# bit-bots/SoccerDiffusion

Hardware: AMD Instinct MI355X
Metric: denoised joint-trajectories/s (50-step DDIM, H=100, J=20) (higher is better)
Workload: dtype f32 (operands split into fp16 hi+lo, 3 fp16 MFMAs per product at every site, fp32 accumulate: 22-bit operands; single noise prediction vs the fp64 oracle 8e-7 on these weights and 2e-6 on weights stressed to |logit| ~ 60 (tests/test_gpu_denoiser.py::test_mode3_noise_prediction_single_step); valid fo; 1 GPU; BASELINE.json configs[2]: 50-step DDIM sampling, B=4096 parallel rollouts per GPU, transformer denoiser d=256 L=4 heads=4, horizon T=100, J=20, memory M=11 (10 context tokens + step token); one step = one full rollout; the timed region issues the rollout's launches eagerly.  Kernel selection: sampler mode 3 (--sampler-mode); batch_per_gpu=4096, ddim_steps=50, horizon=100, joints=20, hidden_dim=256, decoder_layers=4, parallelism=dp1 (independent rollouts, no collective)

## Files before the change

soccerdiffusion_amd/csrc/sd_common.h:

```cpp
#ifndef SD_COMMON_H
#define SD_COMMON_H

#include <hip/hip_runtime.h>
#include <stdint.h>
#include <stdio.h>
#include <atomic>
#include <type_traits>
#include <vector>

#include "../../include/soccerdiffusion_hip.h"

typedef float f32x16 __attribute__((ext_vector_type(16)));
typedef float f32x4 __attribute__((ext_vector_type(4)));

#define SD_LN_EPS 1e-5f

#ifndef SD_PLAIN_STORES
#define SD_PLAIN_STORES 0
#endif
#if SD_PLAIN_STORES
#define SD_NT_STORE(v, p) (*(p) = (v))
#else
#define SD_NT_STORE(v, p) __builtin_nontemporal_store((v), (p))
#endif
// ... 2 lines not shown

#define SD_CHECK_LAUNCH(name)                                 \
    do {                                                      \
        hipError_t e_ = hipGetLastError();                    \
        if (e_ != hipSuccess) return fail((int)e_, name);     \
    } while (0)
#define SD_LAUNCH(...)                    \
    do {                                  \
        (void)hipGetLastError();          \
        hipLaunchKernelGGL(__VA_ARGS__);  \
    } while (0)

struct DevFlag {
    static constexpr int MAX_DEV = 64;
    std::atomic<bool> f[MAX_DEV];
    DevFlag() { for (auto &x : f) x.store(false, std::memory_order_relaxed); }
    static int dev() {
        int d = 0;
        if (hipGetDevice(&d) != hipSuccess || d < 0 || d >= MAX_DEV) d = 0;
        return d;
    }
    bool operator!() const { return !f[dev()].load(std::memory_order_acquire); }
    DevFlag &operator=(bool v) {
        f[dev()].store(v, std::memory_order_release);
        return *this;
    }
};

struct ProfRec { int cls; hipEvent_t a, b; };
struct ProfScope {
    bool on;
    ProfRec rec;
    hipStream_t st;
    ProfScope(int cls, hipStream_t s);
    ~ProfScope();
};

__device__ __forceinline__ float wave_sum(float v) {
#pragma unroll
    for (int o = 32; o > 0; o >>= 1) v += __shfl_xor(v, o, 64);
    return v;
}
__device__ __forceinline__ float wave_max(float v) {
#pragma unroll
    for (int o = 32; o > 0; o >>= 1) v = fmaxf(v, __shfl_xor(v, o, 64));
    return v;
}

__device__ __forceinline__ float row16_sum(float v) {
    v += __builtin_bit_cast(float, __builtin_amdgcn_update_dpp(0, __builtin_bit_cast(int, v), 0x128, 0xF, 0xF, false));
    v += __builtin_bit_cast(float, __builtin_amdgcn_update_dpp(0, __builtin_bit_cast(int, v), 0x124, 0xF, 0xF, false));
    v += __builtin_bit_cast(float, __builtin_amdgcn_update_dpp(0, __builtin_bit_cast(int, v), 0x122, 0xF, 0xF, false));
    v += __builtin_bit_cast(float, __builtin_amdgcn_update_dpp(0, __builtin_bit_cast(int, v), 0x121, 0xF, 0xF, false));
    return v;
}
__device__ __forceinline__ float row16_max(float v) {
    v = fmaxf(v, __builtin_bit_cast(float, __builtin_amdgcn_update_dpp(0, __builtin_bit_cast(int, v), 0x128, 0xF, 0xF, false)));
    v = fmaxf(v, __builtin_bit_cast(float, __builtin_amdgcn_update_dpp(0, __builtin_bit_cast(int, v), 0x124, 0xF, 0xF, false)));
    v = fmaxf(v, __builtin_bit_cast(float, __builtin_amdgcn_update_dpp(0, __builtin_bit_cast(int, v), 0x122, 0xF, 0xF, false)));
    v = fmaxf(v, __builtin_bit_cast(float, __builtin_amdgcn_update_dpp(0, __builtin_bit_cast(int, v), 0x121, 0xF, 0xF, false)));
    return v;
}

__device__ __forceinline__ void quad_transpose(float &x0, float &x1, float &x2, float &x3, int lane) {
    const bool o1 = lane & 1, o2 = lane & 2;
    float ta = o1 ? x0 : x1, tb = o1 ? x2 : x3;
    ta = __builtin_bit_cast(float, __builtin_amdgcn_update_dpp(0, __builtin_bit_cast(int, ta), 0xB1, 0xF, 0xF, false));
    tb = __builtin_bit_cast(float, __builtin_amdgcn_update_dpp(0, __builtin_bit_cast(int, tb), 0xB1, 0xF, 0xF, false));
    if (o1) { x0 = ta; x2 = tb; } else { x1 = ta; x3 = tb; }
    float tc = o2 ? x0 : x2, td = o2 ? x1 : x3;
    tc = __builtin_bit_cast(float, __builtin_amdgcn_update_dpp(0, __builtin_bit_cast(int, tc), 0x4E, 0xF, 0xF, false));
    td = __builtin_bit_cast(float, __builtin_amdgcn_update_dpp(0, __builtin_bit_cast(int, td), 0x4E, 0xF, 0xF, false));
    if (o2) { x0 = tc; x1 = td; } else { x2 = tc; x3 = td; }
}

__device__ __forceinline__ float gelu_erf(float u) { return 0.5f * u * (1.0f + erff(u * 0.70710678118654752440f)); }

__device__ __forceinline__ float gelu_erf_fast(float u) {
    const float z = u * 0.70710678118654752440f, a = fabsf(z);
    const float t = __builtin_amdgcn_rcpf(fmaf(0.5f, a, 1.0f));
    float p = 0.17087277f;
    p = fmaf(p, t, -0.82215223f);
    p = fmaf(p, t, 1.48851587f);
    p = fmaf(p, t, -1.13520398f);
    p = fmaf(p, t, 0.27886807f);
    p = fmaf(p, t, -0.18628806f);
    p = fmaf(p, t, 0.09678418f);
    p = fmaf(p, t, 0.37409196f);
    p = fmaf(p, t, 1.00002368f);
    p = fmaf(p, t, -1.26551223f);
    const float e = t * __builtin_amdgcn_exp2f(fmaf(-a, a, p) * 1.44269504088896340736f);
    return 0.5f * u * (z >= 0.f ? 2.0f - e : e);
}

__device__ __forceinline__ float gelu_grad_fast(float u) {
    const float z = u * 0.70710678118654752440f, a = fabsf(z);
    const float t = __builtin_amdgcn_rcpf(fmaf(0.5f, a, 1.0f));
    float p = 0.17087277f;
    p = fmaf(p, t, -0.82215223f);
    p = fmaf(p, t, 1.48851587f);
    p = fmaf(p, t, -1.13520398f);
    p = fmaf(p, t, 0.27886807f);
    p = fmaf(p, t, -0.18628806f);
    p = fmaf(p, t, 0.09678418f);
    p = fmaf(p, t, 0.37409196f);
    p = fmaf(p, t, 1.00002368f);
    p = fmaf(p, t, -1.26551223f);
    const float g = __builtin_amdgcn_exp2f(-a * a * 1.44269504088896340736f);
    const float e = 0.5f * t * g * __builtin_amdgcn_exp2f(p * 1.44269504088896340736f);
    return (z >= 0.f ? 1.0f - e : e) + u * 0.39894228040143267794f * g;
}

typedef _Float16 f16;
typedef _Float16 f16x4 __attribute__((ext_vector_type(4)));
typedef _Float16 f16x8 __attribute__((ext_vector_type(8)));

typedef float f32x2 __attribute__((ext_vector_type(2)));
__device__ __forceinline__ f32x2 gelu_erf_fast2(f32x2 u) {
    const f32x2 z = u * 0.70710678118654752440f;
    const f32x2 a = {fabsf(z[0]), fabsf(z[1])};
    const f32x2 d = a * 0.5f + 1.0f;
    const f32x2 t = {__builtin_amdgcn_rcpf(d[0]), __builtin_amdgcn_rcpf(d[1])};
    f32x2 p = {0.17087277f, 0.17087277f};
    p = p * t + (-0.82215223f);
    p = p * t + 1.48851587f;
    p = p * t + (-1.13520398f);
    p = p * t + 0.27886807f;
    p = p * t + (-0.18628806f);
    p = p * t + 0.09678418f;
    p = p * t + 0.37409196f;
    p = p * t + 1.00002368f;
    p = p * t + (-1.26551223f);
    const f32x2 x = (p - a * a) * 1.44269504088896340736f;
    const f32x2 e = {t[0] * __builtin_amdgcn_exp2f(x[0]), t[1] * __builtin_amdgcn_exp2f(x[1])};
    const f32x2 w = {z[0] >= 0.f ? 2.0f - e[0] : e[0], z[1] >= 0.f ? 2.0f - e[1] : e[1]};
    return u * 0.5f * w;
}

__device__ __forceinline__ f32x2 gelu_erf_as2(f32x2 u) {
    const f32x2 z = f32x2{fabsf(u[0]), fabsf(u[1])} * 0.70710678118654752440f;
    const f32x2 d = z * 0.3275911f + 1.0f;
    const f32x2 t = {__builtin_amdgcn_rcpf(d[0]), __builtin_amdgcn_rcpf(d[1])};
    f32x2 p = t * 1.061405429f + (-1.453152027f);
    p = p * t + 1.421413741f;
    p = p * t + (-0.284496736f);
    p = p * t + 0.254829592f;
    p = p * t;
    const f32x2 x = z * z * (-1.44269504088896340736f);
    const f32x2 e = {p[0] * __builtin_amdgcn_exp2f(x[0]), p[1] * __builtin_amdgcn_exp2f(x[1])};
    const f32x2 hu = u * 0.5f;
    return f32x2{u[0] >= 0.f ? fmaf(-hu[0], e[0], u[0]) : hu[0] * e[0], u[1] >= 0.f ? fmaf(-hu[1], e[1], u[1]) : hu[1] * e[1]};
}

__device__ __forceinline__ void f16_split4(const f32x4 &x, float scale, f16x4 &h, f16x4 &l) {
#pragma unroll
    for (int e = 0; e < 4; ++e) {
        const float v = x[e] * scale;
        h[e] = (f16)v;
        l[e] = (f16)(v - (float)h[e]);
    }
}

typedef __fp16 fp16x2_t __attribute__((ext_vector_type(2)));
__device__ __forceinline__ void f16_split4_pk(const f32x4 &x, float scale, f16x4 &h, f16x4 &l) {
    const f32x2 a = f32x2{x[0], x[1]} * scale, b = f32x2{x[2], x[3]} * scale;
    const fp16x2_t ha = __builtin_amdgcn_cvt_pkrtz(a[0], a[1]), hb = __builtin_amdgcn_cvt_pkrtz(b[0], b[1]);
    const f32x2 ra = a - f32x2{(float)ha[0], (float)ha[1]}, rb = b - f32x2{(float)hb[0], (float)hb[1]};
    const fp16x2_t la = __builtin_amdgcn_cvt_pkrtz(ra[0], ra[1]), lb = __builtin_amdgcn_cvt_pkrtz(rb[0], rb[1]);
    typedef unsigned u32x2 __attribute__((ext_vector_type(2)));
    h = __builtin_bit_cast(f16x4, u32x2{__builtin_bit_cast(unsigned, ha), __builtin_bit_cast(unsigned, hb)});
    l = __builtin_bit_cast(f16x4, u32x2{__builtin_bit_cast(unsigned, la), __builtin_bit_cast(unsigned, lb)});
}

__device__ __forceinline__ float f16_scale_from_bits(unsigned maxbits) {
    const unsigned eb = (maxbits >> 23) & 0xffu;
    const unsigned sbits = (267u - eb) << 23;
    return (eb >= 14u && eb != 255u) ? __builtin_bit_cast(float, sbits) : 1.0f;
}

struct DropoutArgs {
    unsigned thresh;
    float scale;
    unsigned seed_lo, seed_hi, site_lo, site_hi;
    const unsigned *epoch;
};
extern const unsigned *g_dropout_epoch;

static inline DropoutArgs make_dropout(float p, uint64_t seed, uint64_t site) {
    DropoutArgs a;
    double t = (double)p * 4294967296.0;
    a.thresh = p <= 0.f ? 0u : (t >= 4294967295.0 ? 4294967295u : (unsigned)t);
    a.scale = p <= 0.f ? 1.0f : 1.0f / (1.0f - p);
    a.seed_lo = (unsigned)seed; a.seed_hi = (unsigned)(seed >> 32);
    a.site_lo = (unsigned)site; a.site_hi = (unsigned)(site >> 32);
    a.epoch = g_dropout_epoch;
    return a;
}

__device__ __forceinline__ void philox4x32_7(unsigned c0, unsigned c1, unsigned c2, unsigned c3, unsigned k0, unsigned k1,
                                              unsigned (&w)[4]) {
#pragma unroll
    for (int i = 0; i < 7; ++i) {
        const unsigned long p0 = (unsigned long)0xD2511F53u * (unsigned long)c0, p1 = (unsigned long)0xCD9E8D57u * (unsigned long)c2;
        const unsigned hi0 = (unsigned)(p0 >> 32), lo0 = (unsigned)p0, hi1 = (unsigned)(p1 >> 32), lo1 = (unsigned)p1;
        c0 = hi1 ^ c1 ^ k0;
        c1 = lo1;
        c2 = hi0 ^ c3 ^ k1;
        c3 = lo0;
        k0 += 0x9E3779B9u;
        k1 += 0xBB67AE85u;
    }
    w[0] = c0; w[1] = c1; w[2] = c2; w[3] = c3;
}

__device__ __forceinline__ f32x4 dropout_quad(const DropoutArgs &a, unsigned long quad) {
#ifdef SD_ABL_NOPHILOX
    return f32x4{a.scale, a.scale, a.scale, a.scale} + (float)(quad == 0x123456789ul);
#endif
    unsigned w[4];
    philox4x32_7((unsigned)quad, (unsigned)(quad >> 32), a.site_lo, a.site_hi, a.seed_lo, a.seed_hi + (a.epoch ? *a.epoch : 0u), w);
    f32x4 m;
#pragma unroll
    for (int e = 0; e < 4; ++e) m[e] = w[e] >= a.thresh ? a.scale : 0.f;
    return m;
}

struct PinArgs {
    const float *x0, *noise;
    const int *rows;
};

struct HoldArgs {
    const float *x0, *noise;
    const int *mask;
};

struct MultistepArgs {
    float *hist;
    float w;
};

struct LimitArgs {
    const float *lo, *hi;
    int reproject;
};
__device__ __forceinline__ float limit_update(float x, float e, float lo, float hi, float c0, float c1, float c2, float c3, int reproject, float &x0c) {
    const float x0 = __builtin_fmaf(-c1, e, x) / c0;
    x0c = x0 < lo ? lo : (x0 > hi ? hi : x0);
    if (reproject && !(x0c == x0)) e = __builtin_fmaf(-c0, x0c, x) / c1;
    return __builtin_fmaf(c2, x0c, c3 * e);
}

struct SlewArgs {
    const float *v;
    const float *start;
};
__device__ __forceinline__ float slew_row(float x0, float y, float v, float lo, float hi, bool held, float known) {
    const float a = y - v, c = y + v;
    float z = x0 < a ? a : (x0 > c ? c : x0);
    z = z < lo ? lo : (z > hi ? hi : z);
    return held ? known : z;
}
__device__ __forceinline__ float slew_update(float x, float e, float x0, float x0c, float c0, float c1, float c2, float c3, int reproject) {
    if (reproject && !(x0c == x0)) e = __builtin_fmaf(-c0, x0c, x) / c1;
    return __builtin_fmaf(c2, x0c, c3 * e);
}

struct StepReq {
    float *x, *eps;
    int B, T, Mc;
    int i, n_tok;
    const float *coef;
    bool per_traj;
    int32_t *status;
    const PinArgs *pin;
    int draws;
    const HoldArgs *hold = nullptr;
    const MultistepArgs *ms = nullptr;
    const LimitArgs *lim = nullptr;
    const SlewArgs *slew = nullptr;
};

template <int MAX, class F>
auto by_ntt(int ntt, F f) -> decltype(f(std::integral_constant<int, 1>{})) {
    static_assert(MAX >= 1 && MAX <= 7, "tile counts 1 .. 7 (a horizon of at most 112 rows)");
    switch (ntt) {
        case 1: return f(std::integral_constant<int, 1>{});
        case 2: if constexpr (MAX >= 2) return f(std::integral_constant<int, 2>{}); break;
        case 3: if constexpr (MAX >= 3) return f(std::integral_constant<int, 3>{}); break;
        case 4: if constexpr (MAX >= 4) return f(std::integral_constant<int, 4>{}); break;
        case 5: if constexpr (MAX >= 5) return f(std::integral_constant<int, 5>{}); break;
        case 6: if constexpr (MAX >= 6) return f(std::integral_constant<int, 6>{}); break;
        case 7: if constexpr (MAX >= 7) return f(std::integral_constant<int, 7>{}); break;
        default: break;
    }
    return nullptr;
}

template <class Fn, class... Args>
int launch_step_kernel(Fn fn, const char *name, DevFlag &attr_set, int max_lds, int B, int threads, size_t lds, hipStream_t st, const Args &...args) {
    if (!fn) return fail(SD_E_BADARG, name);
    ProfScope prof(SD_KCLASS_TRAJ_STEP, st);
    if (!attr_set) {
        const hipError_t e = hipFuncSetAttribute((const void *)fn, hipFuncAttributeMaxDynamicSharedMemorySize, max_lds);
        if (e != hipSuccess) {
            static thread_local char msg[128];
// ... 32 lines not shown
```

soccerdiffusion_amd/csrc/sd_traj.h:

```cpp
#pragma once
#include "sd_common.h"
#include "sd_mfma16.h"
#include "soccerdiffusion_hip.h"
#include <type_traits>

namespace tj {

constexpr int D = 256, HD = 64, NH = 4, TMAX = 100;
constexpr int NTHREADS = 512;
constexpr int MAX_L = 8;
constexpr float ACT = 8.0f;
constexpr float PSC = 1024.0f;
constexpr float XSC = 1.0f;
constexpr int XROW = 1024, X1ROW = 512, QROW = 256, VROW = 288, PROW = 512;
constexpr int LDS_X = 0;
constexpr int LDS_SQ = LDS_X + TMAX * X1ROW;
constexpr int LDS_SO = LDS_SQ + TMAX * QROW;
constexpr int LDS_Q = LDS_X + TMAX * XROW;
constexpr int LDS_K = LDS_Q + TMAX * QROW;
constexpr int LDS_P = LDS_Q;
constexpr int LDS_STAT = LDS_K + TMAX * VROW;
constexpr int LDS_BYTES = LDS_STAT + TMAX * 8 * 8;
static_assert(LDS_SO + TMAX * QROW <= LDS_Q, "Q and O fit the freed half of the panel");
static_assert(LDS_BYTES <= 163840 && LDS_P + TMAX * PROW <= LDS_STAT, "LDS budget");
// ... 1008 lines not shown
    {
        const Ctx &c = c0;
        const float s_o = L.sc[0], up = ACT * s_o;
        scale_h(H, up);
        Bias2 bo;
        const SaW sw{L.w_in, L.b_in, L.w_o, L.sc[3], scale_log2e, status};
        if constexpr (PRECISE) sa_block_precise(c, sw, H, L.b_o, bo);
        else sa_block(c, sw, H, L.b_o, bo);
        unscale_h(H, 1.0f / up, bo);
    }
    TJ_STAMP(31);
    LnAffine aff2;
    ln_affine_load(c0, L.n2_w, L.n2_b, aff2);
    float sc4 = 0.f, sc5 = 0.f, sc6 = 0.f, sc7 = 0.f;
    if constexpr (!WIDE) {
        sc4 = L.sc[4], sc5 = L.sc[5], sc6 = L.sc[6], sc7 = L.sc[7];
    }
    f16x8 gfr[8][2];
    if constexpr (!WIDE) {
        const int hh = c0.w >> 1, Mc = Mk - 1;
        const f16 *gp = c0.t == Mc ? gstep + (long)hh * (8 * 2 * 32) + c0.g * 8 : L.g16 + (traj * 4 + hh) * (8 * 2 * 512) + c0.lane * 8;
        const int gstride = c0.t == Mc ? 32 : 512;
        __builtin_amdgcn_sched_barrier(0);
#pragma unroll
        for (int ks = 0; ks < 8; ++ks)
#pragma unroll
            for (int pl = 0; pl < 2; ++pl) gfr[ks][pl] = *reinterpret_cast<const f16x8 *>(gp + (ks * 2 + pl) * gstride);
        __builtin_amdgcn_sched_barrier(0);
    }
    layer_norm_to_x(c0, H, aff2);
    TJ_STAMP(32);
    if constexpr (WIDE) {
        cross_wide(c0, L, H, traj, Mk, nkt, scale_log2e, sblk);
    } else {
        const Ctx c = ctx_local(c0);
        const int hh = c.w >> 1, Mc = Mk - 1;
        const bool odd = c.w & 1;
        const int tt1 = odd ? NH0 : 0, n1 = odd ? NTT - NH0 : NH0;
        char *Pb = c.smem + LDS_P;
        const char *X = c.smem + LDS_X;
        f32x4 S[NH0];
#pragma unroll
        for (int i = 0; i < NH0; ++i) S[i] = f32x4{0.f, 0.f, 0.f, 0.f};
        const auto uni = [](float v) __attribute__((always_inline)) { return __builtin_bit_cast(float, __builtin_amdgcn_readfirstlane(__builtin_bit_cast(int, v))); };
        sc4 = uni(sc4), sc5 = uni(sc5), sc6 = uni(sc6), sc7 = uni(sc7);
        f32x4 cbv = *reinterpret_cast<const f32x4 *>(L.cb + traj * 64 + hh * 16 + 4 * c.g);
        const float cs = L.cstep[sblk * 4 + hh];
        __builtin_amdgcn_sched_barrier(0);
        f16x8 av[2][3][2];
        f16 svv[2][2];
#pragma unroll
        for (int n = 0; n < 2; ++n) {
            const f16 *vp = L.v16 + ((traj * 16 + 2 * c.w + n) * 2) * (2 * 512) + c.lane * 8;
#pragma unroll
            for (int kk = 0; kk < 2; ++kk)
#pragma unroll
                for (int pl = 0; pl < 2; ++pl) av[n][kk][pl] = *reinterpret_cast<const f16x8 *>(vp + (kk * 2 + pl) * 512);
#pragma unroll
            for (int pl = 0; pl < 2; ++pl) svv[n][pl] = vstep[(pl * 4 + c.g) * D + 16 * (2 * c.w + n) + c.t];
        }
        __builtin_amdgcn_sched_barrier(0);
        auto scores = [&](auto odd_c) __attribute__((always_inline)) {
            constexpr bool OD = decltype(odd_c)::value;
            constexpr int N1 = OD ? NTT - NH0 : NH0, T1 = OD ? NH0 : 0;
            constexpr int N1D = N1 > 0 ? N1 : 1;
            f16x8 xb[3][2];
            ring_pipe<8 * N1, 3>(
                [&](int s) __attribute__((always_inline)) {
                    xb[s % 3][0] = lds16(X + x_at(c, T1 + s % N1D, 0, s / N1D));
                    xb[s % 3][1] = lds16(X + x_at(c, T1 + s % N1D, 1, s / N1D));
                },
                [&](int s) __attribute__((always_inline)) { mma3<S_XSC>(S[s % N1D], gfr[s / N1D][0], gfr[s / N1D][1], xb[s % 3][0], xb[s % 3][1]); });
        };
        TJ_WAIT_FIRST_KEY();
        TJ_STAMP(53);
        if (odd) scores(std::true_type{});
        else scores(std::false_type{});
#pragma unroll
        for (int n = 0; n < 2; ++n)
#pragma unroll
            for (int pl = 0; pl < 2; ++pl) av[n][2][pl] = f16x8{svv[n][pl], 0, 0, 0, 0, 0, 0, 0};
        const float c_g = 1.0f / (ACT * sc4);
        const StepScale ss = step_scale(sc5, sc6, sc7);
        f32x4 cg4 = {c_g, c_g, c_g, c_g};
#pragma unroll
        for (int r = 0; r < 4; ++r)
            if (4 * c.g + r == Mc) {
                cbv[r] = cs;
                cg4[r] = ss.c_gs;
            }
        TJ_SYNC(4);
#pragma unroll
        for (int i = 0; i < NH0; ++i) {
            if (i >= n1) continue;
            f32x4 v = S[i] * cg4 + cbv;
#pragma unroll
            for (int r = 0; r < 4; ++r)
                if (4 * c.g + r >= Mk) v[r] = -INFINITY;
            const float m = rows4_max(fmaxf(fmaxf(v[0], v[1]), fmaxf(v[2], v[3])));
            const f32x4 e = (v - m) * scale_log2e;
            f32x4 p = {__builtin_amdgcn_exp2f(e[0]), __builtin_amdgcn_exp2f(e[1]), __builtin_amdgcn_exp2f(e[2]), __builtin_amdgcn_exp2f(e[3])};
            const float sum = rows4_sum((p[0] + p[1]) + (p[2] + p[3]));
            const float f = PSC / sum;
            const float pstep = p[Mc & 3] * (f * ss.m_s);
            p = p * (f * ss.m_c);
            const int tt = tt1 + i, tok = tt < NTT - 1 ? 16 * tt + c.t : c.tok6;
            if (tt == NTT - 1 && !c.ok6) continue;
            const int chunk = (2 * (hh & 1) + (c.g >> 1)) | ((hh >> 1) << 3);
            split_store(Pb + p_off(tok, chunk) + 8 * (c.g & 1), Pb + p_off(tok, chunk | 4) + 8 * (c.g & 1), p);
            if (c.g == (Mc >> 2)) {
                const float pv = pstep;
                const f16 ph = (f16)pv, pl = (f16)(pv - (float)ph);
                const f16x8 z8h = {ph, 0, 0, 0, 0, 0, 0, 0}, z8l = {pl, 0, 0, 0, 0, 0, 0, 0};
                *reinterpret_cast<f16x8 *>(Pb + p_off(tok, hh | (2 << 3))) = z8h;
                *reinterpret_cast<f16x8 *>(Pb + p_off(tok, hh | 4 | (2 << 3))) = z8l;
            }
        }
        TJ_SYNC(5);
        TJ_STAMP(33);
        const float up = PSC * ss.s_v;
        const Bias2 boc = bias_load(c, L.b_oc);
        scale_h(H, up);
        f16x8 pb[3][2];
        ring_pipe<3 * NTT, 3>(
            [&](int s) __attribute__((always_inline)) {
                pb[s % 3][0] = lds16(Pb + p_at(c, s / 3, 0, s % 3));
                pb[s % 3][1] = lds16(Pb + p_at(c, s / 3, 1, s % 3));
            },
            [&](int s) __attribute__((always_inline)) {
                const int tt = s / 3, kk = s % 3;
                mma3<S_XPV>(H[0][tt], av[0][kk][0], av[0][kk][1], pb[s % 3][0], pb[s % 3][1]);
                mma3<S_XPV>(H[1][tt], av[1][kk][0], av[1][kk][1], pb[s % 3][0], pb[s % 3][1]);
            });
        unscale_h(H, 1.0f / up, boc);
    }
    TJ_STAMP(34);
    layer_norm_to_x(c0, H, L.n3_w, L.n3_b);
    TJ_STAMP(35);
    {
        const Ctx c = ctx_local(c0);
        f32x4 U[2][NTT];
#pragma unroll
        for (int a = 0; a < 2; ++a)
#pragma unroll
            for (int tt = 0; tt < NTT; ++tt) U[a][tt] = f32x4{0.f, 0.f, 0.f, 0.f};
        const float sc1 = L.sc[1];
        const Bias2 b1 = bias_load(c, L.b_1);
        gemm_x2<S_W1>(c, U, L.w_1);
        TJ_STAMP(36);
        const float c1 = 1.0f / (ACT * sc1);
        const float sc2 = L.sc[2];
        const Bias2 b2 = bias_load(c, L.b_2);
        TJ_SYNC(6);
#pragma unroll
        for (int tt = 0; tt < NTT; ++tt) {
            f32x4 gl[2];
#pragma unroll
            for (int a = 0; a < 2; ++a) {
                const f32x4 pre = U[a][tt] * c1 + b1.v[a];
                const f32x2 g0 = gelu_erf_as2(f32x2{pre[0], pre[1]}) * ACT, g1 = gelu_erf_as2(f32x2{pre[2], pre[3]}) * ACT;
                gl[a] = f32x4{g0[0], g0[1], g1[0], g1[1]};
            }
            store_x(c, tt, gl[0], gl[1]);
            __builtin_amdgcn_sched_barrier(0);
        }
        TJ_SYNC(7);
        TJ_STAMP(37);
        const float up = ACT * sc2;
        scale_h(H, up);
        gemm_x2<S_W2>(c, H, L.w_2);
        unscale_h(H, 1.0f / up, b2);
    }
    TJ_STAMP(38);
    if (L.nln_w) layer_norm_to_x<!PRECISE>(c0, H, L.nln_w, L.nln_b);
    TJ_STAMP(39);
}

static __device__ __forceinline__ float ddim_update(float x, float e, const f32x4 &k) {
    const float x0 = __builtin_fmaf(-k[1], e, x) / k[0];
    const float ce = k[3] * e;
    return __builtin_fmaf(k[2], x0, ce);
}

template <bool WIDE = false, int PIN = 0, bool ROLL = false, bool DRAWS = false>
static __device__ __forceinline__ void step_body(const StepArgs &a, const PinArgs &pin = PinArgs{}, f32x4 roll_coef = f32x4{0.f, 0.f, 0.f, 0.f},
                                                 int roll_step = 0, int roll_wave = 0, int draws = 1, const HoldArgs &hold = HoldArgs{},
                                                 const MultistepArgs &ms = MultistepArgs{}, const LimitArgs &lim = LimitArgs{},
                                                 const SlewArgs &sl = SlewArgs{}) {
    constexpr bool HOLD = PIN == 2;
    constexpr bool MS = PIN == 3;
    constexpr bool LIM = PIN == 4;
    constexpr bool SLEW = PIN == 5;
    static_assert(!SLEW || TMAX * 128 + TMAX * 4 <= LDS_STAT - LDS_Q, "the slew twin's S and M planes fit the Q | K region");
    extern __shared__ __attribute__((aligned(16))) char smem[];
    Ctx c;
    if constexpr (ROLL) c = ctx_fresh(smem, roll_wave, a.T);
    else ctx_init(c, smem, a.T);
    const long traj = blockIdx.x;
    const long cidx = DRAWS ? (long)((unsigned)blockIdx.x / (unsigned)draws) : traj;
    const int J = a.J;
    TJ_STAMP(0);
    f32x4 H[2][NTT];
    {
        char *Qb = c.smem + LDS_Q;
        f16x8 we[2][2];
        f32x4 be[2], pe4[2][NTT];
#pragma unroll
        for (int n = 0; n < 2; ++n) {
            const f16 *wp = a.w_emb + (long)(2 * c.w + n) * (2 * 512) + c.lane * 8;
            we[n][0] = *reinterpret_cast<const f16x8 *>(wp);
            we[n][1] = *reinterpret_cast<const f16x8 *>(wp + 512);
            const int n0 = 32 * c.w + 16 * n + 4 * c.g;
            be[n] = *reinterpret_cast<const f32x4 *>(a.b_emb + n0);
#pragma unroll
            for (int tt = 0; tt < NTT; ++tt) pe4[n][tt] = *reinterpret_cast<const f32x4 *>(a.pe + (long)tok_of(c, tt) * D + n0);
        }
        __builtin_amdgcn_sched_barrier(0);
        const float *xr = a.x + traj * (long)a.T * J;
        const int tid = ROLL ? 64 * c.w + c.lane : (int)threadIdx.x;
        if (J & 3) {
            for (int i = tid; i < a.T * 4; i += NTHREADS) {
                const int tok = i >> 2, chunk = i & 3;
                f16x8 h8, l8;
#pragma unroll
                for (int e = 0; e < 8; ++e) {
                    const int j = 8 * chunk + e;
                    const float v = j < J ? xr[tok * J + j] * XSC : 0.f;
                    h8[e] = (f16)v;
                    l8[e] = (f16)(v - (float)h8[e]);
                }
                *reinterpret_cast<f16x8 *>(Qb + q_off(tok, chunk)) = h8;
                *reinterpret_cast<f16x8 *>(Qb + q_off(tok, chunk | 4)) = l8;
            }
        }
        const int nvec = (J & 3) ? 0 : a.T * J / 4;
        for (int i = tid; i < nvec; i += NTHREADS) {
            const f32x4 v = *reinterpret_cast<const f32x4 *>(xr + 4 * i) * XSC;
            const int tok = (4 * i) / J, j0 = 4 * i - tok * J;
            const int chunk = j0 >> 3;
            split_store(Qb + q_off(tok, chunk) + 2 * (j0 & 7), Qb + q_off(tok, chunk | 4) + 2 * (j0 & 7), v);
            if (j0 + 4 >= J) {
                const f16x4 z4 = {0, 0, 0, 0};
                for (int k = J; k < 32; k += 4) {
                    *reinterpret_cast<f16x4 *>(Qb + q_off(tok, k >> 3) + 2 * (k & 7)) = z4;
                    *reinterpret_cast<f16x4 *>(Qb + q_off(tok, (k >> 3) | 4) + 2 * (k & 7)) = z4;
                }
            }
        }
        TJ_SYNC(8);
        const float c_e = 1.0f / (XSC * a.sc_io[0]);
#pragma unroll
        for (int n = 0; n < 2; ++n) {
            const f16x8 ah = we[n][0], al = we[n][1];
#pragma unroll
            for (int tt = 0; tt < NTT; ++tt) {
                f32x4 acc = {0.f, 0.f, 0.f, 0.f};
                mma3<S_EMB>(acc, ah, al, lds16(Qb + q_at(c, tt, 0, 0)), lds16(Qb + q_at(c, tt, 1, 0)));
                H[n][tt] = acc * c_e + (be[n] + pe4[n][tt]);
            }
        }
    }
    TJ_STAMP(1);
    layer_norm_to_x<!PRECISE>(c, H, a.n1_w, a.n1_b);
    TJ_STAMP(2);
#pragma unroll 1
    for (int l = 0; l < a.L; ++l) decoder_layer<WIDE>(c, a.layer[l], H, cidx, a.Mk, a.scale_log2e, a.status, a.nkt,
                                                           ROLL ? (long)roll_step : a.step_per_traj ? (a.step_map ? (long)a.step_map[traj] : traj) : 0L);
    const Ctx &c_step = c;
    {
        Ctx c_tail;
        if constexpr (ROLL) c_tail = ctx_fresh(smem, roll_wave, a.T);
        const Ctx &c = ROLL ? c_tail : c_step;
        float *stat = reinterpret_cast<float *>(c.smem + LDS_STAT);
        int pin_rows = 0;
        if constexpr (PIN == 1) pin_rows = (!DRAWS || pin.rows) ? pin.rows[traj] : 0;
        float am[NTT];
#pragma unroll
        for (int tt = 0; tt < NTT; ++tt) {
            const f32x4 a0 = H[0][tt], a1 = H[1][tt];
            float m = fmaxf(fmaxf(fabsf(a0[0]), fabsf(a0[1])), fmaxf(fabsf(a0[2]), fabsf(a0[3])));
            m = fmaxf(m, fmaxf(fmaxf(fabsf(a1[0]), fabsf(a1[1])), fmaxf(fabsf(a1[2]), fabsf(a1[3]))));
            am[tt] = rows4_max(m);
        }
        if (c.g == 0) {
#pragma unroll
            for (int tt = 0; tt < NTT; ++tt)
                if (tok_ok(c, tt)) stat[tok_of(c, tt) * 8 + c.w] = am[tt];
        }
        TJ_SYNC(9);
#pragma unroll
        for (int tt = 0; tt < NTT; ++tt) {
            const float *sp = stat + tok_of(c, tt) * 8;
            const f32x4 p0 = *reinterpret_cast<const f32x4 *>(sp), p1 = *reinterpret_cast<const f32x4 *>(sp + 4);
            const float m = fmaxf(fmaxf(fmaxf(p0[0], p0[1]), fmaxf(p0[2], p0[3])), fmaxf(fmaxf(p1[0], p1[1]), fmaxf(p1[2], p1[3])));
            const float s = f16_scale_from_bits(__builtin_bit_cast(unsigned, m));
            store_x(c, tt, H[0][tt] * s, H[1][tt] * s);
        }
        f16x8 wf[2][8][2];
        if (c.w < NTT) {
#pragma unroll
            for (int n = 0; n < 2; ++n)
#pragma unroll
                for (int ks = 0; ks < 8; ++ks)
#pragma unroll
                    for (int pl = 0; pl < 2; ++pl) wf[n][ks][pl] = *reinterpret_cast<const f16x8 *>(a.w_out + ((long)(n * 8 + ks) * 2 + pl) * 512 + c.lane * 8);
        }
        f32x4 xpre[2] = {f32x4{0.f, 0.f, 0.f, 0.f}, f32x4{0.f, 0.f, 0.f, 0.f}};
        if constexpr (ROLL) {
            if (c.w < NTT && !(J & 3) && (c.w < NTT - 1 || c.ok6)) {
                const int tok = c.w < NTT - 1 ? 16 * c.w + c.t : c.tok6;
#pragma unroll
                for (int n = 0; n < 2; ++n)
                    if (16 * n + 4 * c.g < J) xpre[n] = *reinterpret_cast<const f32x4 *>(a.x + (traj * a.T + tok) * J + 16 * n + 4 * c.g);
            }
        }
        unsigned hold_m = 0;
        if constexpr (HOLD) {
            if (c.w < NTT && (c.w < NTT - 1 || c.ok6)) hold_m = (unsigned)hold.mask[traj * a.T + (c.w < NTT - 1 ? 16 * c.w + c.t : c.tok6)];
        }
        f32x4 hpre[2] = {f32x4{0.f, 0.f, 0.f, 0.f}, f32x4{0.f, 0.f, 0.f, 0.f}};
        if constexpr (MS) {
            if (c.w < NTT && (c.w < NTT - 1 || c.ok6)) {
                const int tok = c.w < NTT - 1 ? 16 * c.w + c.t : c.tok6;
                if (hold.mask) hold_m = (unsigned)hold.mask[traj * a.T + tok];
                if (ms.w != 0.f && !(J & 3)) {
#pragma unroll
                    for (int n = 0; n < 2; ++n)
                        if (16 * n + 4 * c.g < J) hpre[n] = *reinterpret_cast<const f32x4 *>(ms.hist + (traj * a.T + tok) * J + 16 * n + 4 * c.g);
                }
            }
        }
        f32x4 lo4[2] = {f32x4{0.f, 0.f, 0.f, 0.f}, f32x4{0.f, 0.f, 0.f, 0.f}}, hi4[2] = {lo4[0], lo4[0]};
        if constexpr (LIM || SLEW) {
            if (c.w < NTT && (c.w < NTT - 1 || c.ok6)) {
                const int tok = c.w < NTT - 1 ? 16 * c.w + c.t : c.tok6;
                if (hold.mask) hold_m = (unsigned)hold.mask[traj * a.T + tok];
#pragma unroll
                for (int n = 0; n < 2; ++n) {
                    if constexpr (LIM) {
                        lo4[n] = *reinterpret_cast<const f32x4 *>(lim.lo + 16 * n + 4 * c.g);
                        hi4[n] = *reinterpret_cast<const f32x4 *>(lim.hi + 16 * n + 4 * c.g);
                    }
                    if (ms.w != 0.f && !(J & 3) && 16 * n + 4 * c.g < J)
                        hpre[n] = *reinterpret_cast<const f32x4 *>(ms.hist + (traj * a.T + tok) * J + 16 * n + 4 * c.g);
                }
            }
        }
        float scan_v = 0.f, scan_lo = 0.f, scan_hi = 0.f, scan_y = __builtin_nanf("");
        if constexpr (SLEW) {
            if (c.w == 0 && c.lane < J) {
                scan_v = sl.v[c.lane];
                scan_lo = lim.lo[c.lane];
                scan_hi = lim.hi[c.lane];
                if (sl.start) scan_y = sl.start[traj * 32 + c.lane];
            }
        }
        __builtin_amdgcn_sched_barrier(0);
        TJ_SYNC(10);
        if constexpr (SLEW) {
            float *S = reinterpret_cast<float *>(c.smem + LDS_Q);
            unsigned *M = reinterpret_cast<unsigned *>(c.smem + LDS_Q + TMAX * 128);
            const int tok = c.w < NTT - 1 ? 16 * c.w + c.t : c.tok6;
            const bool ok = c.w < NTT && (c.w < NTT - 1 || c.ok6);
            const bool vec = !(J & 3);
            f32x4 ev[2] = {f32x4{0.f, 0.f, 0.f, 0.f}, f32x4{0.f, 0.f, 0.f, 0.f}}, xv[2] = {ev[0], ev[0]}, x0v[2] = {ev[0], ev[0]};
            if (c.w < NTT) {
                const char *X = c.smem + LDS_X;
                f32x4 E[2] = {f32x4{0.f, 0.f, 0.f, 0.f}, f32x4{0.f, 0.f, 0.f, 0.f}};
#pragma unroll
                for (int ks = 0; ks < 8; ++ks) {
                    const int m2lo = (ks & 1) << 1;
                    const unsigned b0 = (c.w < NTT - 1 ? c.xa[m2lo] + (unsigned)(c.w * 16 * XROW) : c.xa6[m2lo]) + (unsigned)((ks >> 1) * 256);
                    const unsigned b1 = (c.w < NTT - 1 ? c.xa[m2lo | 1] + (unsigned)(c.w * 16 * XROW) : c.xa6[m2lo | 1]) + (unsigned)((ks >> 1) * 256);
                    const f16x8 bh = lds16(X + b0), bl = lds16(X + b1);
#pragma unroll
                    for (int n = 0; n < 2; ++n) mma3<S_FC>(E[n], wf[n][ks][0], wf[n][ks][1], bh, bl);
                }
                const float *sp = stat + tok * 8;
                const f32x4 p0 = *reinterpret_cast<const f32x4 *>(sp), p1 = *reinterpret_cast<const f32x4 *>(sp + 4);
                const float m = fmaxf(fmaxf(fmaxf(p0[0], p0[1]), fmaxf(p0[2], p0[3])), fmaxf(fmaxf(p1[0], p1[1]), fmaxf(p1[2], p1[3])));
                const float c_o = 1.0f / (f16_scale_from_bits(__builtin_bit_cast(unsigned, m)) * a.sc_io[1]);
                if (ok && c.g == 0) M[tok] = hold_m;
#pragma unroll
                for (int n = 0; n < 2; ++n) {
                    const int j0 = 16 * n + 4 * c.g;
                    if (!ok || j0 >= J) continue;
                    const long at = (traj * a.T + tok) * J + j0;
                    if (vec) {
// ... 88 lines not shown
            const float *sp = stat + tok * 8;
            const f32x4 p0 = *reinterpret_cast<const f32x4 *>(sp), p1 = *reinterpret_cast<const f32x4 *>(sp + 4);
            const float m = fmaxf(fmaxf(fmaxf(p0[0], p0[1]), fmaxf(p0[2], p0[3])), fmaxf(fmaxf(p1[0], p1[1]), fmaxf(p1[2], p1[3])));
            const float c_o = 1.0f / (f16_scale_from_bits(__builtin_bit_cast(unsigned, m)) * a.sc_io[1]);
#pragma unroll
            for (int n = 0; n < 2; ++n) {
                const int j0 = 16 * n + 4 * c.g;
                if (!ok || j0 >= J) continue;
                const long at = (traj * a.T + tok) * J + j0;
                bool pinned = false;
                if constexpr (PIN == 1) pinned = tok < pin_rows;
                if (J & 3) {
#pragma unroll
                    for (int r = 0; r < 4; ++r) {
                        if (j0 + r >= J) continue;
                        const float e = E[n][r] * c_o + a.b_out[j0 + r];
                        if (a.eps_out) a.eps_out[at + r] = e;
                        if constexpr (PIN == 1) {
                            if (a.update_x && pinned) {
                                a.x[at + r] = a.c2 * pin.x0[at + r] + a.c3 * pin.noise[at + r];
                                continue;
                            }
                        }
                        if constexpr (LIM) {
                            if (a.update_x) {
                                float x0c;
                                float xn = limit_update(a.x[at + r], e, lo4[n][r], hi4[n][r], a.c0, a.c1, a.c2, a.c3, lim.reproject, x0c);
                                if (ms.w != 0.f) xn = __builtin_fmaf(ms.w, ms.hist[at + r] - x0c, xn);
                                if ((hold_m >> (j0 + r)) & 1u) xn = a.c2 * hold.x0[at + r] + a.c3 * hold.noise[at + r];
                                a.x[at + r] = xn;
                                if (ms.hist) ms.hist[at + r] = x0c;
                            }
                            continue;
                        }
                        if constexpr (MS) {
                            if (a.update_x) {
                                const float x0 = __builtin_fmaf(-a.c1, e, a.x[at + r]) / a.c0;
                                float xn = __builtin_fmaf(a.c2, x0, a.c3 * e);
                                if (ms.w != 0.f) xn = __builtin_fmaf(ms.w, ms.hist[at + r] - x0, xn);
                                if ((hold_m >> (j0 + r)) & 1u) xn = a.c2 * hold.x0[at + r] + a.c3 * hold.noise[at + r];
                                a.x[at + r] = xn;
                                ms.hist[at + r] = x0;
                            }
                            continue;
                        }
                        if constexpr (HOLD) {
                            if (a.update_x && ((hold_m >> (j0 + r)) & 1u)) {
                                a.x[at + r] = a.c2 * hold.x0[at + r] + a.c3 * hold.noise[at + r];
                                continue;
                            }
                        }
                        if constexpr (ROLL) {
                            if (a.update_x) a.x[at + r] = ddim_update(a.x[at + r], e, roll_coef);
                            continue;
                        }
                        if (a.update_x) {
                            const float x0 = (a.x[at + r] - a.c1 * e) / a.c0;
                            a.x[at + r] = a.c2 * x0 + a.c3 * e;
                        }
                    }
                    continue;
                }
                const f32x4 e = E[n] * c_o + *reinterpret_cast<const f32x4 *>(a.b_out + j0);
                if (a.eps_out) *reinterpret_cast<f32x4 *>(a.eps_out + at) = e;
                if constexpr (PIN == 1) {
                    if (a.update_x && pinned) {
                        const f32x4 k = *reinterpret_cast<const f32x4 *>(pin.x0 + at), nz = *reinterpret_cast<const f32x4 *>(pin.noise + at);
                        *reinterpret_cast<f32x4 *>(a.x + at) = a.c2 * k + a.c3 * nz;
                        continue;
                    }
                }
                if constexpr (LIM) {
                    if (a.update_x) {
                        const unsigned bits = (hold_m >> j0) & 15u;
                        const f32x4 xv = *reinterpret_cast<const f32x4 *>(a.x + at);
                        f32x4 x0c, xn;
#pragma unroll
                        for (int r = 0; r < 4; ++r) {
                            float q;
                            xn[r] = limit_update(xv[r], e[r], lo4[n][r], hi4[n][r], a.c0, a.c1, a.c2, a.c3, lim.reproject, q);
                            x0c[r] = q;
                        }
                        if (ms.w != 0.f) {
#pragma unroll
                            for (int r = 0; r < 4; ++r) xn[r] = __builtin_fmaf(ms.w, hpre[n][r] - x0c[r], xn[r]);
                        }
                        if (bits) {
                            const f32x4 k = *reinterpret_cast<const f32x4 *>(hold.x0 + at), nz = *reinterpret_cast<const f32x4 *>(hold.noise + at);
                            const f32x4 hv = a.c2 * k + a.c3 * nz;
#pragma unroll
                            for (int r = 0; r < 4; ++r) xn[r] = ((bits >> r) & 1u) ? hv[r] : xn[r];
                        }
                        *reinterpret_cast<f32x4 *>(a.x + at) = xn;
                        if (ms.hist) *reinterpret_cast<f32x4 *>(ms.hist + at) = x0c;
                    }
                    continue;
                }
                if constexpr (MS) {
                    if (a.update_x) {
                        const unsigned bits = (hold_m >> j0) & 15u;
                        const f32x4 xv = *reinterpret_cast<const f32x4 *>(a.x + at);
                        f32x4 x0, xn;
#pragma unroll
                        for (int r = 0; r < 4; ++r) {
                            x0[r] = __builtin_fmaf(-a.c1, e[r], xv[r]) / a.c0;
                            xn[r] = __builtin_fmaf(a.c2, x0[r], a.c3 * e[r]);
                        }
                        if (ms.w != 0.f) {
#pragma unroll
                            for (int r = 0; r < 4; ++r) xn[r] = __builtin_fmaf(ms.w, hpre[n][r] - x0[r], xn[r]);
                        }
                        if (bits) {
                            const f32x4 k = *reinterpret_cast<const f32x4 *>(hold.x0 + at), nz = *reinterpret_cast<const f32x4 *>(hold.noise + at);
                            const f32x4 hv = a.c2 * k + a.c3 * nz;
#pragma unroll
                            for (int r = 0; r < 4; ++r) xn[r] = ((bits >> r) & 1u) ? hv[r] : xn[r];
                        }
                        *reinterpret_cast<f32x4 *>(a.x + at) = xn;
                        *reinterpret_cast<f32x4 *>(ms.hist + at) = x0;
                    }
                    continue;
                }
                if constexpr (HOLD) {
                    const unsigned bits = (hold_m >> j0) & 15u;
                    if (a.update_x && bits) {
                        const f32x4 k = *reinterpret_cast<const f32x4 *>(hold.x0 + at), nz = *reinterpret_cast<const f32x4 *>(hold.noise + at);
                        f32x4 xn = a.c2 * k + a.c3 * nz;
                        if (bits != 15u) {
                            const f32x4 xv = *reinterpret_cast<const f32x4 *>(a.x + at);
#pragma unroll
                            for (int r = 0; r < 4; ++r) {
                                const float x0 = (xv[r] - a.c1 * e[r]) / a.c0;
                                const float u = a.c2 * x0 + a.c3 * e[r];
                                xn[r] = ((bits >> r) & 1u) ? xn[r] : u;
                            }
                        }
                        *reinterpret_cast<f32x4 *>(a.x + at) = xn;
                        continue;
                    }
                }
                if (a.update_x) {
                    const f32x4 xv = ROLL ? xpre[n] : *reinterpret_cast<const f32x4 *>(a.x + at);
                    f32x4 xn;
#pragma unroll
                    for (int r = 0; r < 4; ++r) {
                        if constexpr (ROLL) {
                            xn[r] = ddim_update(xv[r], e[r], roll_coef);
                        } else {
                            const float x0 = (xv[r] - a.c1 * e[r]) / a.c0;
                            xn[r] = a.c2 * x0 + a.c3 * e[r];
                        }
                    }
                    *reinterpret_cast<f32x4 *>(a.x + at) = xn;
                }
            }
        }
    }
    TJ_STAMP(40);
    if constexpr (ROLL) __syncthreads();
}
};

template <int NTT, bool PRECISE>
__global__ __launch_bounds__(NTHREADS, 2) void traj_step_kernel(StepArgs a) { TJ<NTT, PRECISE>::step_body(a); }
template <int NTT>
__global__ __launch_bounds__(NTHREADS, 2) void traj_step_wide_kernel(StepArgs a) { TJ<NTT, true>::template step_body<true>(a); }
template <int NTT>
__global__ __launch_bounds__(NTHREADS, 2) void traj_step_pin_kernel(StepArgs a, PinArgs pin) { TJ<NTT, true>::template step_body<false, true>(a, pin); }
template <int NTT>
__global__ __launch_bounds__(NTHREADS, 2) void traj_step_wide_pin_kernel(StepArgs a, PinArgs pin) { TJ<NTT, true>::template step_body<true, true>(a, pin); }
template <int NTT, bool PRECISE>
__global__ __launch_bounds__(NTHREADS, 2) void traj_step_rollout_kernel(RolloutArgs) {
    typedef const __attribute__((address_space(4))) RolloutArgs *KernArg;
    const int wave = __builtin_amdgcn_readfirstlane(threadIdx.x >> 6);
    const int n_steps = ((KernArg)__builtin_amdgcn_kernarg_segment_ptr())->r.n_steps;
#pragma unroll 1
    for (int i = 0; i < n_steps; ++i) {
        KernArg ka = (KernArg)__builtin_amdgcn_kernarg_segment_ptr();
        asm volatile("" : "+s"(ka));
        const RolloutArgs &k = *(const RolloutArgs *)ka;
        TJ<NTT, PRECISE>::template step_body<false, false, true>(k.a, PinArgs{}, f32x4{k.r.coef[i][0], k.r.coef[i][1], k.r.coef[i][2], k.r.coef[i][3]}, i, wave);
    }
}

template <int NTT, bool PRECISE>
__global__ __launch_bounds__(NTHREADS, 2) void traj_step_draws_kernel(StepArgs a, PinArgs pin, int draws) {
    TJ<NTT, PRECISE>::template step_body<false, true, false, true>(a, pin, f32x4{0.f, 0.f, 0.f, 0.f}, 0, 0, draws);
}
template <int NTT>
__global__ __launch_bounds__(NTHREADS, 2) void traj_step_wide_draws_kernel(StepArgs a, PinArgs pin, int draws) {
    TJ<NTT, true>::template step_body<true, true, false, true>(a, pin, f32x4{0.f, 0.f, 0.f, 0.f}, 0, 0, draws);
}
template <int NTT>
__global__ __launch_bounds__(NTHREADS, 2) void traj_step_hold_kernel(StepArgs a, HoldArgs hold, int draws) {
    TJ<NTT, true>::template step_body<false, 2, false, true>(a, PinArgs{}, f32x4{0.f, 0.f, 0.f, 0.f}, 0, 0, draws, hold);
}
template <int NTT>
__global__ __launch_bounds__(NTHREADS, 2) void traj_step_wide_hold_kernel(StepArgs a, HoldArgs hold, int draws) {
    TJ<NTT, true>::template step_body<true, 2, false, true>(a, PinArgs{}, f32x4{0.f, 0.f, 0.f, 0.f}, 0, 0, draws, hold);
}
template <int NTT>
__global__ __launch_bounds__(NTHREADS, 2) void traj_step_ms_kernel(StepArgs a, HoldArgs hold, MultistepArgs ms, int draws) {
    TJ<NTT, true>::template step_body<false, 3, false, true>(a, PinArgs{}, f32x4{0.f, 0.f, 0.f, 0.f}, 0, 0, draws, hold, ms);
}
template <int NTT>
__global__ __launch_bounds__(NTHREADS, 2) void traj_step_wide_ms_kernel(StepArgs a, HoldArgs hold, MultistepArgs ms, int draws) {
    TJ<NTT, true>::template step_body<true, 3, false, true>(a, PinArgs{}, f32x4{0.f, 0.f, 0.f, 0.f}, 0, 0, draws, hold, ms);
}
template <int NTT>
__global__ __launch_bounds__(NTHREADS, 2) void traj_step_lim_kernel(StepArgs a, HoldArgs hold, MultistepArgs ms, LimitArgs lim, int draws) {
    TJ<NTT, true>::template step_body<false, 4, false, true>(a, PinArgs{}, f32x4{0.f, 0.f, 0.f, 0.f}, 0, 0, draws, hold, ms, lim);
}
template <int NTT>
__global__ __launch_bounds__(NTHREADS, 2) void traj_step_wide_lim_kernel(StepArgs a, HoldArgs hold, MultistepArgs ms, LimitArgs lim, int draws) {
    TJ<NTT, true>::template step_body<true, 4, false, true>(a, PinArgs{}, f32x4{0.f, 0.f, 0.f, 0.f}, 0, 0, draws, hold, ms, lim);
}
template <int NTT>
__global__ __launch_bounds__(NTHREADS, 2) void traj_step_slew_kernel(StepArgs a, HoldArgs hold, MultistepArgs ms, LimitArgs lim, SlewArgs sl, int draws) {
    TJ<NTT, true>::template step_body<false, 5, false, true>(a, PinArgs{}, f32x4{0.f, 0.f, 0.f, 0.f}, 0, 0, draws, hold, ms, lim, sl);
}
template <int NTT>
__global__ __launch_bounds__(NTHREADS, 2) void traj_step_wide_slew_kernel(StepArgs a, HoldArgs hold, MultistepArgs ms, LimitArgs lim, SlewArgs sl, int draws) {
    TJ<NTT, true>::template step_body<true, 5, false, true>(a, PinArgs{}, f32x4{0.f, 0.f, 0.f, 0.f}, 0, 0, draws, hold, ms, lim, sl);
}
struct RolloutDrawsArgs {
    RolloutArgs ra;
    int draws;
};
template <int NTT, bool PRECISE>
__global__ __launch_bounds__(NTHREADS, 2) void traj_step_rollout_draws_kernel(RolloutDrawsArgs) {
    typedef const __attribute__((address_space(4))) RolloutDrawsArgs *KernArg;
    const int wave = __builtin_amdgcn_readfirstlane(threadIdx.x >> 6);
    const int n_steps = ((KernArg)__builtin_amdgcn_kernarg_segment_ptr())->ra.r.n_steps;
#pragma unroll 1
    for (int i = 0; i < n_steps; ++i) {
        KernArg ka = (KernArg)__builtin_amdgcn_kernarg_segment_ptr();
        asm volatile("" : "+s"(ka));
        const RolloutDrawsArgs &k = *(const RolloutDrawsArgs *)ka;
        TJ<NTT, PRECISE>::template step_body<false, false, true, true>(k.ra.a, PinArgs{}, f32x4{k.ra.r.coef[i][0], k.ra.r.coef[i][1], k.ra.r.coef[i][2], k.ra.r.coef[i][3]},
                                                                       i, wave, k.draws);
    }
}

}
```

Measured before the change: 15910 trajectories/s.

## Stage next-step input split in LDS during DDIM update; fold GELU scaling

In the rolled kernel, the DDIM update now writes the new x directly into the LDS Q panel as fp16 hi/lo splits. On later roll steps the start of each step can then skip re-reading x from global memory and re-splitting it. Separately, the ACT scaling is folded into the GELU constants and bias, which removes a few multiplies per element. The staging assumes that the tokens and joints handled in the update match the layout of the input panel and that the LDS Q region survives until the next step.

```diff
diff --git a/soccerdiffusion_amd/csrc/sd_common.h b/soccerdiffusion_amd/csrc/sd_common.h
--- a/soccerdiffusion_amd/csrc/sd_common.h
+++ b/soccerdiffusion_amd/csrc/sd_common.h
@@ -178,6 +178,21 @@
     return f32x2{u[0] >= 0.f ? fmaf(-hu[0], e[0], u[0]) : hu[0] * e[0], u[1] >= 0.f ? fmaf(-hu[1], e[1], u[1]) : hu[1] * e[1]};
 }
 
+template <int S>
+__device__ __forceinline__ f32x2 gelu_erf_as2_scaled(f32x2 su) {
+    const f32x2 z = f32x2{fabsf(su[0]), fabsf(su[1])} * (0.70710678118654752440f / S);
+    const f32x2 d = z * 0.3275911f + 1.0f;
+    const f32x2 t = {__builtin_amdgcn_rcpf(d[0]), __builtin_amdgcn_rcpf(d[1])};
+    f32x2 p = t * (0.5f * 1.061405429f) + (0.5f * -1.453152027f);
+    p = p * t + (0.5f * 1.421413741f);
+    p = p * t + (0.5f * -0.284496736f);
+    p = p * t + (0.5f * 0.254829592f);
+    p = p * t;
+    const f32x2 x = z * z * (-1.44269504088896340736f);
+    const f32x2 e = {p[0] * __builtin_amdgcn_exp2f(x[0]), p[1] * __builtin_amdgcn_exp2f(x[1])};
+    return f32x2{__builtin_fmaf(-fabsf(su[0]), e[0], fmaxf(su[0], 0.f)), __builtin_fmaf(-fabsf(su[1]), e[1], fmaxf(su[1], 0.f))};
+}
+
 __device__ __forceinline__ void f16_split4(const f32x4 &x, float scale, f16x4 &h, f16x4 &l) {
 #pragma unroll
     for (int e = 0; e < 4; ++e) {
diff --git a/soccerdiffusion_amd/csrc/sd_traj.h b/soccerdiffusion_amd/csrc/sd_traj.h
--- a/soccerdiffusion_amd/csrc/sd_traj.h
+++ b/soccerdiffusion_amd/csrc/sd_traj.h
@@ -1184,13 +1184,15 @@
         const float sc2 = L.sc[2];
         const Bias2 b2 = bias_load(c, L.b_2);
         TJ_SYNC(6);
+        const float c1a = c1 * ACT;
+        const f32x4 b1a[2] = {b1.v[0] * ACT, b1.v[1] * ACT};
 #pragma unroll
         for (int tt = 0; tt < NTT; ++tt) {
             f32x4 gl[2];
 #pragma unroll
             for (int a = 0; a < 2; ++a) {
-                const f32x4 pre = U[a][tt] * c1 + b1.v[a];
-                const f32x2 g0 = gelu_erf_as2(f32x2{pre[0], pre[1]}) * ACT, g1 = gelu_erf_as2(f32x2{pre[2], pre[3]}) * ACT;
+                const f32x4 pre = U[a][tt] * c1a + b1a[a];
+                const f32x2 g0 = gelu_erf_as2_scaled<(int)ACT>(f32x2{pre[0], pre[1]}), g1 = gelu_erf_as2_scaled<(int)ACT>(f32x2{pre[2], pre[3]});
                 gl[a] = f32x4{g0[0], g0[1], g1[0], g1[1]};
             }
             store_x(c, tt, gl[0], gl[1]);
@@ -1265,7 +1267,8 @@
                 *reinterpret_cast<f16x8 *>(Qb + q_off(tok, chunk | 4)) = l8;
             }
         }
-        const int nvec = (J & 3) ? 0 : a.T * J / 4;
+        const bool staged = ROLL && roll_step > 0 && a.update_x && !(J & 3);
+        const int nvec = ((J & 3) || staged) ? 0 : a.T * J / 4;
         for (int i = tid; i < nvec; i += NTHREADS) {
             const f32x4 v = *reinterpret_cast<const f32x4 *>(xr + 4 * i) * XSC;
             const int tok = (4 * i) / J, j0 = 4 * i - tok * J;
@@ -1660,6 +1663,18 @@
                         }
                     }
                     *reinterpret_cast<f32x4 *>(a.x + at) = xn;
+                    if constexpr (ROLL) {
+                        char *Qb = c.smem + LDS_Q;
+                        const int chunk = j0 >> 3;
+                        split_store(Qb + q_off(tok, chunk) + 2 * (j0 & 7), Qb + q_off(tok, chunk | 4) + 2 * (j0 & 7), xn * XSC);
+                        if (j0 + 4 >= J) {
+                            const f16x4 z4 = {0, 0, 0, 0};
+                            for (int k = J; k < 32; k += 4) {
+                                *reinterpret_cast<f16x4 *>(Qb + q_off(tok, k >> 3) + 2 * (k & 7)) = z4;
+                                *reinterpret_cast<f16x4 *>(Qb + q_off(tok, (k >> 3) | 4) + 2 * (k & 7)) = z4;
+                            }
+                        }
+                    }
                 }
             }
         }
```

Result: no change. 15970 trajectories/s (median of 6 runs) (+0.4%).
